# dblanm/gnn-manip

Hardware: AMD Instinct MI355X
Metric: rollout steps/sec (N particles, 10 MP steps, hidden=128) (higher is better)
Workload: dtype f32; 1 GPU; north_star target: N=100k dense synthetic scene, conn_r=0.015, max_neighbours=20, hidden=128, 10 MP steps; n_particles=100000, hidden=128, edges_last_step=1966056, k_steps=6, candidates_per_gpu=1, parallelism=candidate-parallel x1

## Files before the change

### gnn_manip_amd/csrc/hedge.hip

```cpp
#include <type_traits>
#include "common.h"
#include "mlp.h"
#include "hedge.h"
#include "hmlp.h"
#include "hmma_dev.h"
#include "blocks_dev.h"

namespace gm {

namespace {

constexpr int H = 128;
constexpr int BE = 32;
constexpr int SYS_THREADS = 768;
static_assert(BE == kBlockEdges, "block tables and the systolic kernels agree on the block size");
#ifdef HEDGE_STAMPS
__device__ unsigned long long g_sys_stamps[3 * 32 * 8 + 32];
#define SYS_STAMP(tick, slot)                                                                                         \
    do {                                                                                                              \
        if (blockIdx.x == 0 && jb == 0 && lane0 == 0 && (tick) >= 16 && (tick) < 48) {                                \
            g_sys_stamps[(role * 32 + (tick) - 16) * 8 + (slot)] = __builtin_readcyclecounter();                     \
            if (role == 0 && (slot) == 0) g_sys_stamps[3 * 32 * 8 + (tick) - 16] = __builtin_amdgcn_s_memrealtime(); \
        }                                                                                                             \
    } while (0)
#else
#define SYS_STAMP(tick, slot) do { } while (0)
#endif
constexpr int ST_STREAM_E = 2 | 16, ST_STREAM_AGG = 16;
constexpr int ST_ENC_E = 0;
constexpr int ST_PROJ_Q = 16;
constexpr int LD_SC1 = 16;
constexpr int HW_HEADER_FLOATS = 4;
constexpr int HW_VEC_FLOATS = 5 * H;
constexpr int HW_IMAGE_HALF8 = 3 * 4 * 8 * 2 * 64;


constexpr int TILE_ROW_B = 144;
constexpr int TILE_B = 32 * TILE_ROW_B;
constexpr int IMG_B = 16384;
constexpr int L_E = 0;
constexpr int L_X1 = L_E + 2 * IMG_B;
constexpr int L_X2 = L_X1 + 2 * IMG_B;
constexpr int L_Z = L_X2 + 2 * IMG_B;
constexpr int L_PS = L_Z + 8 * TILE_B;
constexpr int L_ST = L_PS + 4 * TILE_B;
constexpr int L_KM = L_ST + 2 * 32 * 4 * 4;
constexpr int L_KM2 = L_KM + 4 * 32 * 4;
constexpr int L_ZERO_END = L_KM2 + 4 * 32 * 4;
constexpr int L_VEC = L_ZERO_END;
constexpr int DR_SLOTS = 8;
constexpr int L_DR = L_VEC + 4 * H * 4;
constexpr size_t SYS_LDS_BYTES = L_DR + DR_SLOTS * BE * 4;
static_assert(SYS_LDS_BYTES <= 160 * 1024, "LDS budget");

__device__ __forceinline__ int eslot(int n, int kg, int ksbit) { return (n ^ (2 * (ksbit + 2 * kg))) + 32 * kg; }

typedef __amdgpu_buffer_rsrc_t srd_t;
__device__ __forceinline__ srd_t make_srd(const void* base, unsigned bytes) { return __builtin_amdgcn_make_buffer_rsrc(const_cast<void*>(base), 0, bytes, 0x00020000); }
__device__ __forceinline__ floatx4 bld4(srd_t r, unsigned voff, unsigned soff) { return __builtin_bit_cast(floatx4, __builtin_amdgcn_raw_buffer_load_b128(r, voff, soff, 0)); }
template <int NT>
__device__ __forceinline__ floatx4 bld4s(srd_t r, unsigned voff, unsigned soff) { return __builtin_bit_cast(floatx4, __builtin_amdgcn_raw_buffer_load_b128(r, voff, soff, NT)); }
template <int NT>
__device__ __forceinline__ void bst4s(srd_t r, unsigned voff, unsigned soff, floatx4 v) { __builtin_amdgcn_raw_buffer_store_b128(__builtin_bit_cast(uintx4, v), r, voff, soff, NT); }
__device__ __forceinline__ intx4 bldi4(srd_t r, unsigned voff, unsigned soff) { return __builtin_bit_cast(intx4, __builtin_amdgcn_raw_buffer_load_b128(r, voff, soff, 0)); }
__device__ __forceinline__ void bst4(srd_t r, unsigned voff, unsigned soff, floatx4 v) { __builtin_amdgcn_raw_buffer_store_b128(__builtin_bit_cast(uintx4, v), r, voff, soff, 0); }
template <int AUX>
__device__ __forceinline__ void bst1s(srd_t r, unsigned voff, unsigned soff, float v) { __builtin_amdgcn_raw_buffer_store_b32(__float_as_uint(v), r, voff, soff, AUX); }
__device__ __forceinline__ int xcd_major_wg() {
    const int g = (int)gridDim.x, i = (int)blockIdx.x;
    return (g & 7) == 0 ? (i & 7) * (g >> 3) + (i >> 3) : i;
}

__device__ __forceinline__ int s_clamp0(int v, int hi) {
    int r;
    asm("s_max_i32 %0, %1, 0\n\ts_min_i32 %0, %0, %2" : "=s"(r) : "s"(v), "s"(hi) : "scc");
    return r;
}

extern __shared__ __attribute__((aligned(16))) char smem[];
#define LDS(T, off) (*reinterpret_cast<T*>(smem + (off)))
__device__ __forceinline__ unsigned opaque(unsigned v) { asm volatile("" : "+v"(v)); return v; }
__device__ __forceinline__ int tick_no(int t) { asm volatile("" : "+s"(t)); return t; }
#define GM_SB __builtin_amdgcn_sched_barrier(0)

template <int NP>
__device__ __forceinline__ void acc_to_image(const floatx16& a, char* smem, unsigned addr) {
#pragma unroll
    for (int q = 0; q < 2; ++q) {
        float v[8];
#pragma unroll
        for (int j = 0; j < 8; ++j) v[j] = relu(a[8 * q + j]);
        uintx2 h0, l0, h1, l1;
        if constexpr (NP == 3) {
            split4(v[0], v[1], v[2], v[3], h0, l0);
            split4(v[4], v[5], v[6], v[7], h1, l1);
        } else {
            hi4(v[0], v[1], v[2], v[3], h0);
            hi4(v[4], v[5], v[6], v[7], h1);
        }
        LDS(uintx4, addr + (q * 2 + 0) * 1024) = uintx4{h0[0], h0[1], h1[0], h1[1]};
        if constexpr (NP == 3) LDS(uintx4, addr + (q * 2 + 1) * 1024) = uintx4{l0[0], l0[1], l1[0], l1[1]};
    }
}

template <int NP, class F>
__device__ __forceinline__ void mlp_layer(floatx16& acc, const floatx16& c0, const half8 (&wh)[8], const half8 (&wl)[8], char* smem, unsigned a0, unsigned a1, F&& side) {
    if constexpr (NP == 1) {
        half8 bh = LDS(half8, a0);
#pragma unroll
        for (int ks = 0; ks < 8; ++ks) {
            half8 nh = bh;
            const unsigned an = (((ks + 1) & 1) ? a1 : a0) + (ks + 1) * 2048;
            GM_SB;
            acc = __builtin_amdgcn_mfma_f32_32x32x16_f16(wh[ks], bh, ks == 0 ? c0 : acc, 0, 0, 0);
            GM_SB;
            if (ks + 1 < 8) nh = LDS(half8, an);
            side(3 * ks);
            GM_SB;
            side(3 * ks + 1);
            GM_SB;
            side(3 * ks + 2);
            bh = nh;
        }
        GM_SB;
        return;
    }
    half8 bh = LDS(half8, a0), bl = LDS(half8, a0 + 1024);
#pragma unroll
    for (int ks = 0; ks < 8; ++ks) {
        half8 nh = bh;
        const unsigned an = (((ks + 1) & 1) ? a1 : a0) + (ks + 1) * 2048;
        GM_SB;
        acc = __builtin_amdgcn_mfma_f32_32x32x16_f16(wl[ks], bh, ks == 0 ? c0 : acc, 0, 0, 0);
        GM_SB;
        if (ks + 1 < 8) nh = LDS(half8, an);
        side(3 * ks);
        GM_SB;
        acc = __builtin_amdgcn_mfma_f32_32x32x16_f16(wh[ks], bl, acc, 0, 0, 0);
        GM_SB;
        if (ks + 1 < 8) bl = LDS(half8, an + 1024);
        side(3 * ks + 1);
        GM_SB;
        acc = __builtin_amdgcn_mfma_f32_32x32x16_f16(wh[ks], bh, acc, 0, 0, 0);
        GM_SB;
        side(3 * ks + 2);
        bh = nh;
    }
    GM_SB;
}

__device__ __forceinline__ float ln_k(char* smem, unsigned st, float inv_T, float eps) {
    const float q = (LDS(float, st) + LDS(float, st + 128)) + (LDS(float, st + 256) + LDS(float, st + 384));
    const float v = fmaf(q * (1.0f / 128.0f) * inv_T, inv_T, eps);
    float r = __builtin_amdgcn_rsqf(v);
    r = r * fmaf(-0.5f * v * r, r, 1.5f);
    return inv_T * r;
}

__device__ __forceinline__ float lower_half_to_both(float v) {
    const auto r = __builtin_amdgcn_permlane32_swap(__float_as_uint(v), __float_as_uint(v), false, false);
    return __uint_as_float(r[0]);
}
__device__ __forceinline__ float upper_half_to_both(float v) {
    const auto r = __builtin_amdgcn_permlane32_swap(__float_as_uint(v), __float_as_uint(v), false, false);
    return __uint_as_float(r[1]);
}
__device__ __forceinline__ float sum_of_halves(float v) {
    const auto r = __builtin_amdgcn_permlane32_swap(__float_as_uint(v), __float_as_uint(v), false, false);
    return __uint_as_float(r[0]) + __uint_as_float(r[1]);
}

template <int R>
__device__ __forceinline__ void scan3_t(float& ya, float& yb, float& yc, float yprev, unsigned cont) {
    asm volatile("s_bfe_i32 exec_lo, %4, %5\n\ts_bfe_i32 exec_hi, %4, %6\n\tv_add_f32 %0, %0, %3\n\t"
                 "s_bfe_i32 exec_lo, %4, %7\n\ts_bfe_i32 exec_hi, %4, %8\n\tv_add_f32 %1, %1, %0\n\t"
                 "s_bfe_i32 exec_lo, %4, %9\n\ts_bfe_i32 exec_hi, %4, %10\n\tv_add_f32 %2, %2, %1\n\t"
                 "s_mov_b64 exec, -1"
                 : "+v"(ya), "+v"(yb), "+v"(yc)
                 : "v"(yprev), "s"(cont), "n"(0x10000 | R), "n"(0x10000 | (16 + R)), "n"(0x10000 | (R + 1)), "n"(0x10000 | (17 + R)),
// ... 335 lines not shown
        const unsigned km_rq = opaque(L_KM2 + jb * 128 + 64 * hi);
        const unsigned z_w = opaque(L_Z + jb * TILE_B + n * TILE_ROW_B + hi * 16);
        const unsigned z_t = opaque(L_Z + jb * TILE_B + 16 * hi * TILE_ROW_B + n * 4);
        const unsigned x_in = opaque(L_X2 + lane0 * 16);
        const unsigned dr_r = opaque(L_DR + 64 * hi);
        const srd_t srd_agg = make_srd(reinterpret_cast<const char*>(a_agg) - L_ST, a_agg_bytes + L_ST);
        floatx16 b3v = vec_to_acc(smem, L_VEC, H, jb, hi);
        auto fetch = [&](int x, int2 bi, int2 si, int hd, int& st, int& cnt, int& fl, unsigned& cont, unsigned& last, int& head) {
            st = bi.x;
            if (!ok(x)) { cnt = 0; fl = 0; cont = 0; last = 0; return; }
            cnt = bi.y & 0xff;
            fl = bi.y >> 8;
            cont = (unsigned)si.x;
            last = (unsigned)si.y;
            if (fl & 1) head = hd;
        };
        auto tick_as = [&](auto par_c, auto kind_c, int t) __attribute__((always_inline)) {
            constexpr int PAR = decltype(par_c)::value, P2 = PAR, P3 = 1 - PAR;
            constexpr int KIND = decltype(kind_c)::value;
            const int x = b0 + t;
            const int2 bn_n = a_blk[clampb(x)], sn_n = a_seg[clampb(x)];
            const int hd_n = a_head[clampb(x - 1) >> 2];
            if constexpr (KIND == TICK_IDLE) {
                cnt_a = cnt_b; fl_a = fl_b; cont_a = cont_b; last_a = last_b;
                if (fl_b & 1) head_a = head_b;
                st_a = st_b;
                fetch(x - 1, bn, sn, hd_n, st_b, cnt_b, fl_b, cont_b, last_b, head_b);
                bn = bn_n;
                sn = sn_n;
                lds_barrier();
                return;
            }
            b3v = vec_to_acc(smem, L_VEC, H, jb, hi);
            const bool agg_on = ok(x - 3);
            SYS_STAMP(t, 0);
            LDS(float, v_aoff + (L_KM2 - L_ST)) = ln_k(smem, st_r + P3 * 512, inv_T, a_eps);
            SYS_STAMP(t, 1);
            const unsigned cont = agg_on ? cont_a : 0u, last = agg_on ? last_a : 0u;
            const int cnt_st = agg_on ? cnt_a : 0;
            const unsigned rel_a = (unsigned)(st_a - e0), rel_b = (unsigned)(st_b - e0);
            floatx16 y;
            floatx4 kq;
            float zz[4];
            LnGroup lg;
            float cpend = 0.f;
            auto side = [&](int slot) {
                if (slot < 8) {
                    const int c = slot >> 1;
                    if (!(slot & 1)) {
                        kq = LDS(floatx4, km_rq + 16 * c);
#pragma unroll
                        for (int i = 0; i < 4; ++i) zz[i] = LDS(float, z_t + P3 * 4 * TILE_B + (4 * c + i) * TILE_ROW_B);
                    } else {
#pragma unroll
                        for (int i = 0; i < 4; ++i) y[4 * c + i] = fmaf(zz[i] * kq[i], gam, bet);
                    }
                } else if (slot < 13) {
                    const int r = 3 * (slot - 8) + 1;
                    float ya = y[r], yb = y[r + 1], yc = y[r + 2];
                    const float yp = y[r - 1];
                    scan3(ya, yb, yc, yp, cont, r);
                    y[r] = ya; y[r + 1] = yb; y[r + 2] = yc;
                } else if (slot == 13) {
                    const float c0v = (cont & 1u) ? carry : 0.f;
                    const float open0 = y[15] + ((last & 0xffffu) ? 0.f : c0v);
                    const float from0 = lower_half_to_both(open0);
                    const float c1v = (cont & 0x10000u) ? from0 : 0.f;
                    cpend = hi ? c1v : c0v;
                } else if (WRITE_E && slot >= 14 && slot < 20) {
                    const int j = 1 + ((slot - 14) >> 1);
                    if (!((slot - 14) & 1)) {
                        lg.load(km_re + j * 32, z_e + P3 * 4 * TILE_B + j * 8 * TILE_ROW_B);
                    } else {
                        const floatx4 gmq = LDS(floatx4, L_VEC + (2 * H + 32 * jb + 4 * cq) * 4);
                        const floatx4 btq = LDS(floatx4, L_VEC + (3 * H + 32 * jb + 4 * cq) * 4);
                        lg.store<STREAM ? ST_STREAM_E : 0>(e_out_wg, rel_a, j, cnt_st, v_eoff, gmq, btq, er[j - 1], res_w, srd_ein, rel_b);
                    }
                }
            };
            SYS_STAMP(t, 2);
            auto stores = [&]() {
                unsigned pend = (last | (last >> 16)) & 0xffffu;
                const unsigned side_row = (a_side_off + (unsigned)(((x - 3) >> 2) * H)) * 4u;
                const unsigned drp = dr_r + ((x - 3) & (DR_SLOTS - 1)) * (BE * 4);
                while (pend) {
                    const int r = __builtin_ctz(pend);
                    pend &= pend - 1;
                    const unsigned long long mk = (unsigned long long)(0u - ((last >> r) & 1u)) | ((unsigned long long)(0u - ((last >> (16 + r)) & 1u)) << 32);
                    if (__builtin_amdgcn_inverse_ballot_w64(mk)) {
                        const int d = LDS(int, drp + 4 * r);
                        const unsigned off = (d == head_a ? side_row : (unsigned)d * (H * 4u)) + v_aoff;
                        bst1s<STREAM ? ST_STREAM_AGG : 0>(srd_agg, off, 0, y[r] + cpend);
                        cpend = 0.f;
                    }
                }
                const float nc = upper_half_to_both(y[15] + cpend);
                carry = (((last >> 31) & 1u) || !agg_on || cnt_a < BE) ? 0.f : nc;
            };
            if constexpr (KIND == TICK_DRAIN) {
#pragma unroll
                for (int slot = 0; slot < 20; ++slot) side(slot);
            } else {
            mlp_layer<NP>(acc, b3v, wh, wl, smem, x_in + P2 * IMG_B, x_in + P2 * IMG_B, side);
            SYS_STAMP(t, 3);
            rng |= __any(row_bad<NP>(acc[0])) ? 1 : 0;
            {
                float q = 0.f;
#pragma unroll
                for (int r = 0; r < 16; ++r) q = fmaf(acc[r], acc[r], q);
                LDS(float, v_aoff + P2 * 512) = sum_of_halves(q);
#pragma unroll
                for (int g = 0; g < 4; ++g) {
                    floatx4 z;
#pragma unroll
                    for (int tt = 0; tt < 4; ++tt) z[tt] = acc[4 * g + tt];
                    LDS(floatx4, z_w + P2 * 4 * TILE_B + 32 * g) = z;
                }
            }
            }
            SYS_STAMP(t, 4);
            stores();
            cnt_a = cnt_b; fl_a = fl_b; cont_a = cont_b; last_a = last_b;
            if (fl_b & 1) head_a = head_b;
            st_a = st_b;
            fetch(x - 1, bn, sn, hd_n, st_b, cnt_b, fl_b, cont_b, last_b, head_b);
            bn = bn_n;
            sn = sn_n;
            SYS_STAMP(t, 5);
            lds_barrier();
            SYS_STAMP(t, 6);
        };
        auto tick = [&](auto par_c, int t) __attribute__((always_inline)) { tick_as(par_c, int_c<TICK_FULL>{}, t); };
        tick_as(int_c<1>{}, int_c<TICK_IDLE>{}, -1);
        tick_as(int_c<0>{}, int_c<TICK_IDLE>{}, 0);
        tick_as(int_c<1>{}, int_c<TICK_IDLE>{}, 1);
        tick(int_c<0>{}, tick_no(2));
        RUN_TICKS(3, nb - 1, tick);
        tick(int_c<1>{}, nb + 1);
        tick_as(int_c<0>{}, int_c<TICK_DRAIN>{}, nb + 2);
        report_split_range<false>(rng, lane0, a_flags);
    }
}

constexpr int LE_X1 = 0;
constexpr int LE_X2 = LE_X1 + 2 * IMG_B;
constexpr int LE_Z = LE_X2 + 2 * IMG_B;
constexpr int LE_ST = LE_Z + 8 * TILE_B;
constexpr int LE_KM = LE_ST + 2 * 4 * 32 * 4;
constexpr int RS_SLOTS = 8;
constexpr int LE_RS = LE_KM + 4 * 32 * 4;
constexpr int LE_ZERO_END = LE_RS + RS_SLOTS * 32 * 4;
constexpr int LE_VEC = LE_ZERO_END;
constexpr size_t ENC_LDS_BYTES = LE_VEC + 5 * H * 4;

template <int NP>
__global__ void __launch_bounds__(SYS_THREADS, 1) sys_enc_kernel(const CsrHeader* a_hdr, const float* __restrict__ a_x, float* __restrict__ a_e_out,
                                                                      const float* __restrict__ a_hw, int* a_flags, float a_eps, int a_pad_rows) {
    const int tid = threadIdx.x, lane0 = tid & 63;
    const int wave = __builtin_amdgcn_readfirstlane(tid >> 6);
    const int role = wave >> 2, jb = wave & 3;
    const int E = a_hdr->n_edges;
    const int nblk = (E + BE - 1) / BE;
    const int2 br = wg_range(nblk, true);
    const int b0 = br.x, b1 = br.y;
    const int nb = b1 - b0;
    if (a_pad_rows && blockIdx.x == 0)
        for (int i = tid; i < kEdgePadRows * H / 4; i += SYS_THREADS) reinterpret_cast<floatx4*>(a_e_out + (size_t)E * H)[i] = floatx4{0.f, 0.f, 0.f, 0.f};
    if (nb <= 0) return;
    const float inv_T = a_hw[1], cap = a_hw[2];
    half8 wh[8], wl[8];
    sys_prologue<NP>(wh, wl, reinterpret_cast<const half8*>(a_hw + HW_HEADER_FLOATS + HW_VEC_FLOATS), role * 4 + jb, role == 0, LE_ZERO_END, LE_VEC,
                      a_hw + HW_HEADER_FLOATS, 5 * H);
    const int n = lane0 & 31, hi = lane0 >> 5, rr = lane0 >> 3, cq = lane0 & 7;
    const int e0 = b0 * BE;
    const int rows_wg = (b1 * BE < E ? b1 * BE : E) - e0;
    floatx16 bv;
    {
        const int slot = role == 0 ? 4 : role - 1;
#pragma unroll
        for (int g = 0; g < 4; ++g) {
            const floatx4 v = LDS(floatx4, LE_VEC + (slot * H + 32 * jb + 4 * hi + 8 * g) * 4);
#pragma unroll
            for (int tt = 0; tt < 4; ++tt) bv[4 * g + tt] = v[tt];
        }
    }
    const unsigned rs_l = opaque(LE_RS + n * 4);
    int rng = 0;
    floatx16 acc;
    auto scaled_bias = [&](float sc) {
        floatx16 c;
#pragma unroll
        for (int r = 0; r < 16; ++r) c[r] = bv[r] * sc;
        return c;
    };
    if (role == 0) {
        const srd_t srd_x = make_srd(a_x + (size_t)e0 * 4, (unsigned)(rows_wg > 0 ? rows_wg : 0) * 16u);
        float* const e_out_wg = a_e_out + (size_t)e0 * H;
        const unsigned v_xoff = opaque(n * 16 + (hi ? 0x40000000u : 0u));
        const unsigned v_eoff = opaque(rr * 512 + jb * 128 + cq * 16);
        const unsigned x1_w = opaque(LE_X1 + 4 * jb * 1024 + lane0 * 16);
        const unsigned st_r = opaque(LE_ST + n * 4);
        const unsigned km_w = opaque(LE_KM + jb * 128 + n * 4), km_r = opaque(LE_KM + jb * 128 + rr * 4);
        const unsigned z_r = opaque(LE_Z + jb * TILE_B + rr * TILE_ROW_B + cq * 16);
        const floatx4 gm = LDS(floatx4, LE_VEC + (2 * H + 32 * jb + 4 * cq) * 4);
        const floatx4 bt = LDS(floatx4, LE_VEC + (3 * H + 32 * jb + 4 * cq) * 4);
        const float T3 = 1.0f / inv_T;
        floatx4 xq = bld4(srd_x, v_xoff, 0);
        auto tick = [&](auto par_c, int t) {
            constexpr int PAR = decltype(par_c)::value, P3 = 1 - PAR;
            const int x = b0 + t;
            float mx = fmaxf(fmaxf(fabsf(xq[0]), fabsf(xq[1])), fmaxf(fabsf(xq[2]), fabsf(xq[3])));
            float sc = cap;
            if (mx > 0.f && mx < 3.0e38f) {
                int ex;
                (void)frexpf(mx, &ex);
                sc = fminf(ldexpf(1.f, min(7 - ex, 100)), cap);
            }
            sc = lower_half_to_both(sc);
            if (jb == 0 && hi == 0) LDS(float, rs_l + (x & (RS_SLOTS - 1)) * 128) = sc;
            uintx2 h, l;
            if constexpr (NP == 3) split4(xq[0] * sc, xq[1] * sc, xq[2] * sc, xq[3] * sc, h, l);
            else hi4(xq[0] * sc, xq[1] * sc, xq[2] * sc, xq[3] * sc, h);
            const half8 bh = __builtin_bit_cast(half8, uintx4{h[0], h[1], 0u, 0u});
            const floatx16 c0v = scaled_bias(sc);
            {
                const int xn = x + 1 < b0 ? b0 : (x + 1 < b1 ? x + 1 : b1 - 1);
                xq = bld4(srd_x, v_xoff, (unsigned)(xn - b0) * 512u);
            }
            if constexpr (NP == 3) {
            const half8 bl = __builtin_bit_cast(half8, uintx4{l[0], l[1], 0u, 0u});
            acc = __builtin_amdgcn_mfma_f32_32x32x16_f16(wl[0], bh, c0v, 0, 0, 0);
            acc = __builtin_amdgcn_mfma_f32_32x32x16_f16(wh[0], bl, acc, 0, 0, 0);
            acc = __builtin_amdgcn_mfma_f32_32x32x16_f16(wh[0], bh, acc, 0, 0, 0);
            } else {
                acc = __builtin_amdgcn_mfma_f32_32x32x16_f16(wh[0], bh, c0v, 0, 0, 0);
            }
            {
                const float rs3 = LDS(float, rs_l + ((x - 3) & (RS_SLOTS - 1)) * 128);
                const float q = (LDS(float, st_r + P3 * 512) + LDS(float, st_r + P3 * 512 + 128)) + (LDS(float, st_r + P3 * 512 + 256) + LDS(float, st_r + P3 * 512 + 384));
                const float tt3 = T3 * rs3;
                const float v = fmaf(a_eps * tt3, tt3, q * (1.0f / 128.0f));
                float r = __builtin_amdgcn_rsqf(v);
                r = r * fmaf(-0.5f * v * r, r, 1.5f);
                LDS(float, km_w) = r;
                const int xb = x - 3;
                const int cnt = (xb >= b0 && xb < b1) ? min(BE, E - xb * BE) : 0;
#pragma unroll
                for (int j = 0; j < 4; ++j) {
                    const float kr = LDS(float, km_r + j * 32);
                    const floatx4 zq = LDS(floatx4, z_r + P3 * 4 * TILE_B + j * 8 * TILE_ROW_B);
                    floatx4 o;
#pragma unroll
                    for (int tt = 0; tt < 4; ++tt) o[tt] = fmaf(zq[tt] * kr, gm[tt], bt[tt]);
                    bst4s<ST_ENC_E>(make_srd(e_out_wg + (size_t)((xb - b0) * BE + 8 * j) * H, (unsigned)s_clamp0(cnt - 8 * j, 8) * 512u), v_eoff, 0, o);
                }
            }
            rng |= __any(row_bad<NP>(acc[0])) ? 1 : 0;
            GM_SB;
            acc_to_image<NP>(acc, smem, x1_w + PAR * IMG_B);
            lds_barrier();
        };
        RUN_TICKS(0, nb + 2, tick);
    } else if (role == 1) {
        const unsigned x_in = opaque(LE_X1 + lane0 * 16), x_out = opaque(LE_X2 + 4 * jb * 1024 + lane0 * 16);
        auto nothing = [](int) {};
        auto tick = [&](auto par_c, int t) {
            constexpr int PAR = decltype(par_c)::value, P1 = 1 - PAR;
            const int x = b0 + t;
            const floatx16 c0v = scaled_bias(LDS(float, rs_l + ((x - 1) & (RS_SLOTS - 1)) * 128));
            mlp_layer<NP>(acc, c0v, wh, wl, smem, x_in + P1 * IMG_B, x_in + P1 * IMG_B, nothing);
            rng |= __any(row_bad<NP>(acc[0])) ? 1 : 0;
            GM_SB;
            acc_to_image<NP>(acc, smem, x_out + P1 * IMG_B);
            lds_barrier();
        };
        RUN_TICKS(0, nb + 2, tick);
    } else {
        const unsigned x_in = opaque(LE_X2 + lane0 * 16);
        const unsigned st_w = opaque(LE_ST + jb * 128 + n * 4);
        const unsigned z_w = opaque(LE_Z + jb * TILE_B + n * TILE_ROW_B + hi * 16);
        auto nothing = [](int) {};
        auto tick = [&](auto par_c, int t) {
            constexpr int PAR = decltype(par_c)::value, P2 = PAR;
            const int x = b0 + t;
            const floatx16 c0v = scaled_bias(LDS(float, rs_l + ((x - 2) & (RS_SLOTS - 1)) * 128));
            mlp_layer<NP>(acc, c0v, wh, wl, smem, x_in + P2 * IMG_B, x_in + P2 * IMG_B, nothing);
            rng |= __any(row_bad<NP>(acc[0])) ? 1 : 0;
            publish_ln_stats(acc, st_w + P2 * 512, z_w + P2 * 4 * TILE_B);
            lds_barrier();
        };
        RUN_TICKS(0, nb + 2, tick);
    }
    report_split_range(rng, lane0, a_flags);
}

constexpr int LN_E = 0;
constexpr int LN_X1 = LN_E + 2 * IMG_B;
constexpr int LN_X2 = LN_X1 + 2 * IMG_B;
constexpr int LN_Z = LN_X2 + 2 * IMG_B;
constexpr int LN_PS = LN_Z + 8 * TILE_B;
constexpr int LN_ST = LN_PS + 4 * TILE_B;
constexpr int LN_KM = LN_ST + 2 * 4 * 32 * 4;
constexpr int LN_ZERO_END = LN_KM + 2 * 4 * 32 * 4;
constexpr int LN_VEC = LN_ZERO_END;
constexpr size_t NODE_LDS_BYTES = LN_VEC + 4 * H * 4;
static_assert(NODE_LDS_BYTES <= 160 * 1024, "LDS budget");

template <int NP>
__device__ __forceinline__ void sys_node_body(const float* a_h, const float* __restrict__ a_agg, const float* __restrict__ a_Q,
                                              float* a_h_out, const float* __restrict__ a_hw, int a_n, int* a_flags, float a_eps) {
    const int tid = threadIdx.x, lane0 = tid & 63;
    const int wave = __builtin_amdgcn_readfirstlane(tid >> 6);
    const int role = wave >> 2, jb = wave & 3;
    const int N = a_n;
    const int nblk = (N + BE - 1) / BE;
    const int wg = (int)blockIdx.x;
    const int b0 = (int)((long long)wg * nblk / gridDim.x), b1 = (int)((long long)(wg + 1) * nblk / gridDim.x);
    const int nb = b1 - b0;
    if (nb <= 0) return;
    const float inv_T = a_hw[1];
    half8 wh[8], wl[8];
    sys_prologue<NP>(wh, wl, reinterpret_cast<const half8*>(a_hw + HW_HEADER_FLOATS + HW_VEC_FLOATS), role * 4 + jb, false, LN_ZERO_END, LN_VEC,
                 a_hw + HW_HEADER_FLOATS, 4 * H);
    const int n = lane0 & 31, hi = lane0 >> 5, rr = lane0 >> 3, cq = lane0 & 7;
    const int r0 = b0 * BE;
    const int rows_wg = (b1 * BE < N ? b1 * BE : N) - r0;
    const unsigned wg_bytes = (unsigned)(rows_wg > 0 ? rows_wg : 0) * 512u;
    const unsigned v_eoff = opaque(rr * 512 + jb * 128 + cq * 16);
    int rng = 0;
    set_role_prio(role);
    if (role == 0) {
        const srd_t srd_q = make_srd(a_Q + (size_t)r0 * H, wg_bytes), srd_a = make_srd(a_agg + (size_t)r0 * H, wg_bytes);
        const unsigned v_qoff = opaque(rr * 2048 + jb * 128 + cq * 16);
        const unsigned ps_w = opaque(LN_PS + jb * TILE_B + 4 * rr * TILE_ROW_B + cq * 16);
        const unsigned ps_r = opaque(LN_PS + jb * TILE_B + n * TILE_ROW_B + hi * 16);
        const int kg = cq & 1, ksb = cq >> 2, half = (cq >> 1) & 1;
        const unsigned e_w = opaque(LN_E + ((2 * jb + ksb) * 2 * 64 + ((rr ^ (2 * (ksb + 2 * kg))) + 32 * kg)) * 16 + half * 8);
        const unsigned e_r0 = opaque(LN_E + eslot(n, hi, 0) * 16), e_r1 = opaque(LN_E + eslot(n, hi, 1) * 16);
        const unsigned x1_w = opaque(LN_X1 + 4 * jb * 1024 + lane0 * 16);
        floatx4 qv[4], eq[4];
#pragma unroll
        for (int j = 0; j < 4; ++j) { qv[j] = floatx4{0.f, 0.f, 0.f, 0.f}; eq[j] = bld4(srd_a, v_eoff, j * 4096); }
        floatx16 acc, c0v;
#pragma unroll
        for (int r = 0; r < 16; ++r) c0v[r] = 0.f;
        auto clampb = [&](int x) { return x < b0 ? b0 : (x < b1 ? x : b1 - 1); };
        auto tick_as = [&](auto par_c, auto kind_c, int t) {
            constexpr int PAR = decltype(par_c)::value, KIND = decltype(kind_c)::value;
            if constexpr (KIND == TICK_DRAIN) {
                lds_barrier();
                return;
            }
            const int x = b0 + t;
            const unsigned rel1 = (unsigned)(clampb(x + 1) - b0) * (BE * 512u), rel2 = (unsigned)(clampb(x + 2) - b0) * (BE * 512u);
#pragma unroll
            for (int j = 0; j < 4; ++j) qv[j] = bld4(srd_q, v_qoff, rel1 + j * 512);
            auto side = [&](int slot) {
                if (slot < 8 && !(slot & 1)) {
                    const int j = slot >> 1;
                    uintx2 h, l;
                    if constexpr (NP == 3) split4(eq[j][0], eq[j][1], eq[j][2], eq[j][3], h, l);
                    else hi4(eq[j][0], eq[j][1], eq[j][2], eq[j][3], h);
                    LDS(uintx2, e_w + (1 - PAR) * IMG_B + j * 128) = h;
                    if constexpr (NP == 3) LDS(uintx2, e_w + (1 - PAR) * IMG_B + j * 128 + 1024) = l;
                } else if (slot == 8) {
#pragma unroll
                    for (int j = 0; j < 4; ++j) eq[j] = bld4(srd_a, v_eoff, rel2 + j * 4096);
                }
            };
            if constexpr (KIND == TICK_FULL) {
                mlp_layer<NP>(acc, c0v, wh, wl, smem, e_r0 + PAR * IMG_B, e_r1 + PAR * IMG_B, side);
                rng |= __any(row_bad<NP>(acc[0])) ? 1 : 0;
                GM_SB;
                acc_to_image<NP>(acc, smem, x1_w + PAR * IMG_B);
            } else {
#pragma unroll
                for (int slot = 0; slot <= 8; ++slot) side(slot);
            }
#pragma unroll
            for (int j = 0; j < 4; ++j) LDS(floatx4, ps_w + j * TILE_ROW_B) = qv[j];
#pragma unroll
            for (int g = 0; g < 4; ++g) {
                const floatx4 v = LDS(floatx4, ps_r + 32 * g);
#pragma unroll
                for (int tt = 0; tt < 4; ++tt) c0v[4 * g + tt] = v[tt];
            }
            lds_barrier();
        };
        NODE_TICKS(tick_as);
    } else {
        const bool r2 = role == 2;
        const int eg0 = r2 ? 2 : 0;
        const srd_t srd_h = make_srd(a_h + (size_t)r0 * H, wg_bytes);
        float* const h_out_wg = a_h_out + (size_t)r0 * H;
        const floatx4 gm = LDS(floatx4, LN_VEC + (2 * H + 32 * jb + 4 * cq) * 4);
        const floatx4 bt = LDS(floatx4, LN_VEC + (3 * H + 32 * jb + 4 * cq) * 4);
        const floatx16 bv = vec_to_acc(smem, LN_VEC, r2 ? H : 0, jb, hi);
        const unsigned st_r = opaque(LN_ST + n * 4);
        const unsigned km_w = opaque(LN_KM + (r2 ? 512 : 0) + jb * 128 + n * 4), km_r = opaque(LN_KM + (r2 ? 512 : 0) + jb * 128 + rr * 4);
        const unsigned z_r = opaque(LN_Z + jb * TILE_B + rr * TILE_ROW_B + cq * 16);
        const unsigned x_in = opaque((r2 ? LN_X2 : LN_X1) + lane0 * 16), x_out = opaque(LN_X2 + 4 * jb * 1024 + lane0 * 16);
        const unsigned st_w = opaque(LN_ST + jb * 128 + n * 4);
        const unsigned z_w = opaque(LN_Z + jb * TILE_B + n * TILE_ROW_B + hi * 16);
        floatx4 er[2];
        er[0] = er[1] = floatx4{0.f, 0.f, 0.f, 0.f};
        floatx16 acc;
        auto tick_as = [&](auto par_c, auto kind_c, int t) {
            constexpr int PAR = decltype(par_c)::value, PIN = 1 - PAR, P3 = 1 - PAR;
            constexpr int KIND = decltype(kind_c)::value;
            if constexpr (KIND == TICK_FILL) {
                lds_barrier();
                return;
            }
            const int x = b0 + t;
            LDS(float, km_w) = ln_k(smem, st_r + P3 * 512, inv_T, a_eps);
            const int xb = x - 3;
            const int cnt = (xb >= b0 && xb < b1) ? min(BE, N - xb * BE) : 0;
            const unsigned rel_a = (unsigned)((xb < b0 ? b0 : xb) - b0) * BE;
            const int xr = x - 2 < b0 ? b0 : (x - 2 < b1 ? x - 2 : b1 - 1);
            const unsigned rel_b = (unsigned)(xr - b0) * (BE * 512u);
            float kr;
            floatx4 zq;
            auto side = [&](int slot) {
                if (slot != 0 && slot != 2 && slot != 6 && slot != 8) return;
                const int jj = slot >= 6, j = eg0 + jj;
                if (slot == 0 || slot == 6) {
                    kr = LDS(float, km_r + j * 32);
                    zq = LDS(floatx4, z_r + P3 * 4 * TILE_B + j * 8 * TILE_ROW_B);
                } else {
                    floatx4 o;
#pragma unroll
                    for (int tt = 0; tt < 4; ++tt) o[tt] = er[jj][tt] + fmaf(zq[tt] * kr, gm[tt], bt[tt]);
                    bst4(make_srd(h_out_wg + (size_t)(rel_a + 8 * j) * H, (unsigned)s_clamp0(cnt - 8 * j, 8) * 512u), v_eoff, 0, o);
                    er[jj] = bld4(srd_h, v_eoff, rel_b + j * 4096);
                }
            };
            if constexpr (KIND == TICK_DRAIN) {
#pragma unroll
                for (int slot = 0; slot <= 8; ++slot) side(slot);
            } else if (!r2) {
                mlp_layer<NP>(acc, bv, wh, wl, smem, x_in + PIN * IMG_B, x_in + PIN * IMG_B, side);
                rng |= __any(row_bad<NP>(acc[0])) ? 1 : 0;
                GM_SB;
                acc_to_image<NP>(acc, smem, x_out + PIN * IMG_B);
// ... 322 lines not shown
        }
        hipLaunchKernelGGL(pack_h3_kernel, dim3(J.n), dim3(H3_PACK_THREADS), 0, s, J);
        GM_LAUNCH_CHECK();
    }
    return GM_OK;
}

static size_t max_blocks_of(int64_t n_nodes, int64_t edge_capacity) {
    return (size_t)cdiv(edge_capacity, BE) + 4 * (size_t)n_nodes + 4;
}
size_t edge_groups_max(int64_t n_nodes, int64_t edge_capacity) { return max_blocks_of(n_nodes, edge_capacity) / 4 + 1 + kSinkRows; }

size_t edge_blocks_ints(int64_t n_nodes, int64_t edge_capacity) {
    const size_t nblk = max_blocks_of(n_nodes, edge_capacity);
    return 8 + ((size_t)n_nodes + 2) + 1 + 4 * nblk + (nblk / 4 + 2) + 2 * (size_t)n_nodes;
}

EdgeBlocks carve_edge_blocks(int* base, int64_t n_nodes, int64_t edge_capacity) {
    EdgeBlocks t;
    const size_t nblk = max_blocks_of(n_nodes, edge_capacity);
    t.hdr = reinterpret_cast<EdgeBlockHeader*>(base);
    t.gblk = base + 8;
    int* p = t.gblk + n_nodes + 2;
    p += (reinterpret_cast<uintptr_t>(p) & 4) ? 1 : 0;
    t.blk = reinterpret_cast<int2*>(p);
    t.seg = reinterpret_cast<int2*>(p + 2 * nblk);
    t.head = p + 4 * nblk;
    t.stitch = t.head + nblk / 4 + 2;
    t.stitch_list = t.stitch + n_nodes;
    t.max_blocks = (int64_t)nblk;
    return t;
}

int build_edge_blocks(const int* in_ptr, const int* dst, int64_t n_nodes, const int* n_per_graph_dev, int n_per_graph_host, const EdgeBlocks& t, hipStream_t s) {
    hipLaunchKernelGGL(edge_blocks_plan_kernel, dim3(1), dim3(64), 0, s, in_ptr, (int)n_nodes, n_per_graph_dev, n_per_graph_host,
                       t.hdr, t.gblk, (int)n_nodes + 1);
    int gb = (int)cdiv(t.max_blocks, 256);
    gb = gb < 1 ? 1 : (gb > 1024 ? 1024 : gb);
    hipLaunchKernelGGL(edge_blocks_fill_kernel, dim3(gb), dim3(256), 0, s, in_ptr, dst, (int)n_nodes, t.hdr, t.gblk, t.blk, t.seg, t.head, t.stitch,
                       t.stitch_list);
    GM_LAUNCH_CHECK();
    return GM_OK;
}

bool edge_sys_fits(int64_t n_nodes, int64_t edge_capacity) {
    const uint64_t agg_rows = (uint64_t)n_nodes + edge_groups_max(n_nodes, edge_capacity);
    return (uint64_t)n_nodes * 2 * H * 4 < (1ull << 32) && agg_rows * H * 4 < (1ull << 32);
}

constexpr uint64_t kStreamStoreBytes = 128ull << 20;

template <auto KERNEL, class... Args>
static int launch_sys(size_t lds, ProfState* prof_state, int kind, hipStream_t s, Args... args) {
    static PerDeviceOnce attr_done;
    const int rc_attr = attr_done.run([lds]() -> int {
        GM_HIP_CHECK(hipFuncSetAttribute(reinterpret_cast<const void*>(KERNEL), hipFuncAttributeMaxDynamicSharedMemorySize, (int)lds));
        return GM_OK;
    });
    if (rc_attr != GM_OK) return rc_attr;
    {
        ProfScope prof(prof_state, kind, s);
        hipLaunchKernelGGL(KERNEL, dim3(device_cus()), dim3(SYS_THREADS), lds, s, args...);
    }
    GM_LAUNCH_CHECK();
    return GM_OK;
}
template <auto KERNEL>
using kernel_c = std::integral_constant<decltype(KERNEL), KERNEL>;
int launch_edge_sys(const EdgeArgs& a, const EdgeBlocks& t, int64_t edge_capacity, hipStream_t s) {
    GM_REQUIRE(a.hdr && a.wstream_h3 && a.agg && a.side && !a.eid && !a.eid_out, GM_ERR_INVALID_ARGUMENT, "launch_edge_sys: unsupported argument combination");
    GM_REQUIRE(a.P_prescaled, GM_ERR_INVALID_ARGUMENT, "launch_edge_sys: P must carry the weight scale of this step (HmNodeArgs::p_scale = edge_sys_p_scale(image))");
    const uint64_t agg_bytes = ((uint64_t)(a.side - a.agg) + (uint64_t)(t.max_blocks / 4 + 1) * H) * 4;
    GM_REQUIRE(a.side >= a.agg && agg_bytes < (1ull << 32) && (uint64_t)a.n_nodes_tab * 2 * H * 4 < (1ull << 32), GM_ERR_INVALID_ARGUMENT,
               "launch_edge_sys: P and agg + side buffer must each stay below 4 GiB (edge_sys_fits)");
    const bool stream = (uint64_t)edge_capacity * H * 4 > kStreamStoreBytes;
    auto go = [&](auto kern) {
        return launch_sys<decltype(kern)::value>(SYS_LDS_BYTES, a.prof, PROF_EDGE, s, a.hdr, a.dst, a.src, a.P, a.e_in, a.e_out, a.agg, a.wstream_h3,
                                                 t.blk, t.seg, t.head, t.hdr, (unsigned)(a.side - a.agg), (unsigned)agg_bytes,
                                                 (unsigned)((uint64_t)a.n_nodes_tab * 2 * H * 4), const_cast<int*>(&a.hdr->error_flags), a.eps, a.residual);
    };
    auto pick = [&](auto np_c) {
        constexpr int NP = decltype(np_c)::value;
        if (a.discard_e_out) return stream ? go(kernel_c<sys_edge_kernel<false, true, NP>>{}) : go(kernel_c<sys_edge_kernel<false, false, NP>>{});
        return stream ? go(kernel_c<sys_edge_kernel<true, true, NP>>{}) : go(kernel_c<sys_edge_kernel<true, false, NP>>{});
    };
    return a.precision == kPrecisionF16 ? pick(int_c<NP_F16>{}) : pick(int_c<NP_F32>{});
}

int launch_edge_sys_enc(const EdgeArgs& a, hipStream_t s) {
    GM_REQUIRE(a.hdr && a.wstream_h3 && a.e_in && a.e_out && !a.eid && !a.eid_out && a.k1 == 4, GM_ERR_INVALID_ARGUMENT,
               "launch_edge_sys_enc: unsupported argument combination");
    auto go = [&](auto kern) {
        return launch_sys<decltype(kern)::value>(ENC_LDS_BYTES, a.prof, PROF_ENC, s, a.hdr, a.e_in, a.e_out, a.wstream_h3, const_cast<int*>(&a.hdr->error_flags),
                                                 a.eps, a.zero_pad_rows ? 1 : 0);
    };
    return a.precision == kPrecisionF16 ? go(kernel_c<sys_enc_kernel<NP_F16>>{}) : go(kernel_c<sys_enc_kernel<NP_F32>>{});
}

int launch_node_sys(const NodeSysArgs& a, hipStream_t s) {
    GM_REQUIRE(a.h && a.agg && a.Q && a.h_out && a.image && a.n > 0, GM_ERR_INVALID_ARGUMENT, "launch_node_sys: bad argument");
    auto go = [&](auto kern) {
        return launch_sys<decltype(kern)::value>(NODE_LDS_BYTES, a.prof, PROF_NODE, s, a.h, a.agg, a.Q, a.h_out, a.image, a.n, a.flags, a.eps);
    };
    return a.precision == kPrecisionF16 ? go(kernel_c<sys_node_kernel<NP_F16>>{}) : go(kernel_c<sys_node_kernel<NP_F32>>{});
}

int launch_proj_sys(const ProjSysArgs& a, hipStream_t s) {
    GM_REQUIRE(a.h && a.P && a.Q && a.img_p && a.img_q && a.n > 0, GM_ERR_INVALID_ARGUMENT, "launch_proj_sys: bad argument");
    auto go = [&](auto kern) {
        return launch_sys<decltype(kern)::value>(PROJ_LDS_BYTES, a.prof, PROF_NODE, s, a.h, a.P, a.Q, a.img_p, a.img_q, a.scale_p, a.scale_q, a.n, a.flags);
    };
    return a.precision == kPrecisionF16 ? go(kernel_c<sys_proj_kernel<NP_F16>>{}) : go(kernel_c<sys_proj_kernel<NP_F32>>{});
}

int launch_node_proj_sys(const NodeSysArgs& a, const ProjSysArgs& p, hipStream_t s) {
    GM_REQUIRE(a.h && a.agg && a.Q && a.h_out && a.image && a.n > 0, GM_ERR_INVALID_ARGUMENT, "launch_node_proj_sys: bad argument");
    GM_REQUIRE(p.P && p.img_p && p.img_q, GM_ERR_INVALID_ARGUMENT, "launch_node_proj_sys: bad argument");
    GM_REQUIRE(p.h == a.h_out && p.Q == a.Q && p.n == a.n && p.flags == a.flags, GM_ERR_INVALID_ARGUMENT,
               "launch_node_proj_sys: the projection must read the node MLP's h_out and write its Q, over the same rows");
    GM_REQUIRE(p.precision == a.precision, GM_ERR_INVALID_ARGUMENT, "launch_node_proj_sys: the two halves disagree on the precision");
    auto go = [&](auto kern) {
        return launch_sys<decltype(kern)::value>(NODE_PROJ_LDS_BYTES, a.prof, PROF_NODE, s, a.h, a.h_out, a.agg, p.Q, a.image, p.P, p.img_p, p.img_q,
                                                 p.scale_p, p.scale_q, a.n, a.flags, a.eps);
    };
    return a.precision == kPrecisionF16 ? go(kernel_c<sys_node_proj_kernel<NP_F16>>{}) : go(kernel_c<sys_node_proj_kernel<NP_F32>>{});
}

int launch_agg_stitch(float* agg, const float* side, const EdgeBlocks& t, int64_t n, ProfState* prof_state, hipStream_t s) {
    if (n <= 0) return GM_OK;
    {
        ProfScope prof(prof_state, PROF_NODE, s);
        int64_t gb = cdiv(n * 8, 256 * 4);
        gb = gb < 1 ? 1 : (gb > 2048 ? 2048 : gb);
        hipLaunchKernelGGL(agg_stitch_kernel, dim3((unsigned)gb), dim3(256), 0, s, agg, side, t.stitch, t.stitch_list, t.head, t.hdr, (int)n);
    }
    GM_LAUNCH_CHECK();
    return GM_OK;
}

__global__ void __launch_bounds__(256) edge_pad_rows_kernel(const CsrHeader* hdr, float* e, int row_floats) {
    const size_t base = (size_t)hdr->n_edges * row_floats;
    for (int i = blockIdx.x * blockDim.x + threadIdx.x; i < kEdgePadRows * row_floats; i += gridDim.x * blockDim.x) e[base + i] = 0.f;
}
int zero_edge_pad_rows(const CsrHeader* hdr, float* e, int row_floats, hipStream_t s) {
    hipLaunchKernelGGL(edge_pad_rows_kernel, dim3(4), dim3(256), 0, s, hdr, e, row_floats);
    GM_LAUNCH_CHECK();
    return GM_OK;
}

#ifdef HEDGE_STAMPS
extern "C" int gm_debug_sys_stamps(unsigned long long* out) {
    return hipMemcpyFromSymbol(out, HIP_SYMBOL(g_sys_stamps), sizeof(unsigned long long) * (3 * 32 * 8 + 32)) == hipSuccess ? 0 : -1;
}
#endif

}
```

Measured before the change: 128.5 rollout steps/s.

## Deepen edge-encoder systolic pipeline to overlap MLP epilogues with next block's MFMA chain

The three-role edge-encoder kernel moves from a 3-stage to a 5-stage software pipeline. Roles 1 and 2 keep double-buffered accumulators, so the relu/convert/LDS-store epilogue (or the LayerNorm statistics) of the previous block is interleaved as side work inside the next block's MFMA chain. This hides epilogue latency behind matrix ops. In exchange it adds register pressure from two floatx16 accumulators, deeper fill and drain ticks, more complex tick scheduling macros, and debug stamps that are compiled out by default.

```diff
diff --git a/gnn_manip_amd/csrc/hedge.hip b/gnn_manip_amd/csrc/hedge.hip
--- a/gnn_manip_amd/csrc/hedge.hip
+++ b/gnn_manip_amd/csrc/hedge.hip
@@ -23,8 +23,15 @@
             if (role == 0 && (slot) == 0) g_sys_stamps[3 * 32 * 8 + (tick) - 16] = __builtin_amdgcn_s_memrealtime(); \
         }                                                                                                             \
     } while (0)
+__device__ unsigned long long g_enc_stamps[3 * 32 * 8];
+#define ENC_STAMP(tick, slot)                                                                                         \
+    do {                                                                                                              \
+        if (blockIdx.x == 0 && jb == 0 && lane0 == 0 && (tick) >= 16 && (tick) < 48)                                  \
+            g_enc_stamps[(role * 32 + (tick) - 16) * 8 + (slot)] = __builtin_readcyclecounter();                     \
+    } while (0)
 #else
 #define SYS_STAMP(tick, slot) do { } while (0)
+#define ENC_STAMP(tick, slot) do { } while (0)
 #endif
 constexpr int ST_STREAM_E = 2 | 16, ST_STREAM_AGG = 16;
 constexpr int ST_ENC_E = 0;
@@ -666,6 +673,43 @@
 constexpr int LE_ZERO_END = LE_RS + RS_SLOTS * 32 * 4;
 constexpr int LE_VEC = LE_ZERO_END;
 constexpr size_t ENC_LDS_BYTES = LE_VEC + 5 * H * 4;
+static_assert(ENC_LDS_BYTES <= 160 * 1024, "LDS budget");
+constexpr int ENC_DEPTH = 5;
+static_assert(ENC_DEPTH + 1 <= RS_SLOTS, "the scale ring holds every block in flight");
+
+#define ENC_T(tick_as, par, ch, tl, t) tick_as(int_c<(par)>{}, std::bool_constant<(ch)>{}, std::bool_constant<(tl)>{}, t)
+#define ENC_DRAIN(tick_as, C, D, p0)                                \
+    ENC_T(tick_as, (p0), 0 < (C), 0 < (D), nb);                     \
+    ENC_T(tick_as, 1 - (p0), 1 < (C), 1 < (D), nb + 1);             \
+    ENC_T(tick_as, (p0), 2 < (C), 2 < (D), nb + 2);                 \
+    ENC_T(tick_as, 1 - (p0), 3 < (C), 3 < (D), nb + 3);             \
+    ENC_T(tick_as, (p0), 4 < (C), 4 < (D), nb + 4);
+#define ENC_TICKS(tick_as, C, D)                                                                        \
+    if (nb >= ENC_DEPTH) {                                                                              \
+        ENC_T(tick_as, 0, 0 >= (C), 0 >= (D), 0);                                                       \
+        ENC_T(tick_as, 1, 1 >= (C), 1 >= (D), 1);                                                       \
+        ENC_T(tick_as, 0, 2 >= (C), 2 >= (D), 2);                                                       \
+        ENC_T(tick_as, 1, 3 >= (C), 3 >= (D), 3);                                                       \
+        ENC_T(tick_as, 0, 4 >= (C), 4 >= (D), 4);                                                       \
+        int t_ = ENC_DEPTH;                                                                             \
+        _Pragma("unroll 1") for (; t_ + 1 < nb; t_ += 2) {                                              \
+            ENC_T(tick_as, 1, true, true, t_);                                                          \
+            ENC_T(tick_as, 0, true, true, t_ + 1);                                                      \
+        }                                                                                               \
+        if (t_ < nb) {              \
+            ENC_T(tick_as, 1, true, true, t_);                                                          \
+            ENC_DRAIN(tick_as, C, D, 0)                                                                 \
+        } else {                                                                                        \
+            ENC_DRAIN(tick_as, C, D, 1)                                                                 \
+        }                                                                                               \
+    } else {                                                                                            \
+        _Pragma("unroll 1") for (int t_ = 0; t_ < nb + ENC_DEPTH; t_ += 2) {                            \
+            tick_as(int_c<0>{}, t_ >= (C) && t_ < (C) + nb, t_ >= (D) && t_ < (D) + nb, t_);            \
+            if (t_ + 1 < nb + ENC_DEPTH)                                                                \
+                tick_as(int_c<1>{}, t_ + 1 >= (C) && t_ + 1 < (C) + nb, t_ + 1 >= (D) && t_ + 1 < (D) + nb, t_ + 1); \
+        }                                                                                               \
+    }
+static_assert(ENC_DEPTH == 5, "ENC_TICKS and ENC_DRAIN spell out five fill and five drain ticks");
 
 template <int NP>
 __global__ void __launch_bounds__(SYS_THREADS, 1) sys_enc_kernel(const CsrHeader* a_hdr, const float* __restrict__ a_x, float* __restrict__ a_e_out,
@@ -700,14 +744,16 @@
     }
     const unsigned rs_l = opaque(LE_RS + n * 4);
     int rng = 0;
-    floatx16 acc;
+    floatx16 acc2[2];
     auto scaled_bias = [&](float sc) {
         floatx16 c;
 #pragma unroll
         for (int r = 0; r < 16; ++r) c[r] = bv[r] * sc;
         return c;
     };
+    auto nothing = [](int) {};
     if (role == 0) {
+        floatx16& acc = acc2[0];
         const srd_t srd_x = make_srd(a_x + (size_t)e0 * 4, (unsigned)(rows_wg > 0 ? rows_wg : 0) * 16u);
         float* const e_out_wg = a_e_out + (size_t)e0 * H;
         const unsigned v_xoff = opaque(n * 16 + (hi ? 0x40000000u : 0u));
@@ -720,9 +766,12 @@
         const floatx4 bt = LDS(floatx4, LE_VEC + (3 * H + 32 * jb + 4 * cq) * 4);
         const float T3 = 1.0f / inv_T;
         floatx4 xq = bld4(srd_x, v_xoff, 0);
-        auto tick = [&](auto par_c, int t) {
+        auto tick_as = [&](auto par_c, auto ch, auto ep, int t) __attribute__((always_inline)) {
             constexpr int PAR = decltype(par_c)::value, P3 = 1 - PAR;
+            constexpr bool FULL = std::is_same_v<decltype(ch), bool>;
             const int x = b0 + t;
+            ENC_STAMP(t, 0);
+            if (FULL || ch) {
             float mx = fmaxf(fmaxf(fabsf(xq[0]), fabsf(xq[1])), fmaxf(fabsf(xq[2]), fabsf(xq[3])));
             float sc = cap;
             if (mx > 0.f && mx < 3.0e38f) {
@@ -749,15 +798,17 @@
             } else {
                 acc = __builtin_amdgcn_mfma_f32_32x32x16_f16(wh[0], bh, c0v, 0, 0, 0);
             }
-            {
-                const float rs3 = LDS(float, rs_l + ((x - 3) & (RS_SLOTS - 1)) * 128);
+            }
+            ENC_STAMP(t, 1);
+            if (FULL || ep) {
+                const float rs3 = LDS(float, rs_l + ((x - ENC_DEPTH) & (RS_SLOTS - 1)) * 128);
                 const float q = (LDS(float, st_r + P3 * 512) + LDS(float, st_r + P3 * 512 + 128)) + (LDS(float, st_r + P3 * 512 + 256) + LDS(float, st_r + P3 * 512 + 384));
                 const float tt3 = T3 * rs3;
                 const float v = fmaf(a_eps * tt3, tt3, q * (1.0f / 128.0f));
                 float r = __builtin_amdgcn_rsqf(v);
                 r = r * fmaf(-0.5f * v * r, r, 1.5f);
                 LDS(float, km_w) = r;
-                const int xb = x - 3;
+                const int xb = x - ENC_DEPTH;
                 const int cnt = (xb >= b0 && xb < b1) ? min(BE, E - xb * BE) : 0;
 #pragma unroll
                 for (int j = 0; j < 4; ++j) {
@@ -769,41 +820,102 @@
                     bst4s<ST_ENC_E>(make_srd(e_out_wg + (size_t)((xb - b0) * BE + 8 * j) * H, (unsigned)s_clamp0(cnt - 8 * j, 8) * 512u), v_eoff, 0, o);
                 }
             }
-            rng |= __any(row_bad<NP>(acc[0])) ? 1 : 0;
-            GM_SB;
-            acc_to_image<NP>(acc, smem, x1_w + PAR * IMG_B);
+            if (FULL || ch) {
+                rng |= __any(row_bad<NP>(acc[0])) ? 1 : 0;
+                GM_SB;
+                acc_to_image<NP>(acc, smem, x1_w + PAR * IMG_B);
+            }
+            ENC_STAMP(t, 2);
             lds_barrier();
+            ENC_STAMP(t, 3);
         };
-        RUN_TICKS(0, nb + 2, tick);
+        ENC_TICKS(tick_as, 0, ENC_DEPTH)
     } else if (role == 1) {
         const unsigned x_in = opaque(LE_X1 + lane0 * 16), x_out = opaque(LE_X2 + 4 * jb * 1024 + lane0 * 16);
-        auto nothing = [](int) {};
-        auto tick = [&](auto par_c, int t) {
+        auto tick_as = [&](auto par_c, auto ch, auto tl, int t) __attribute__((always_inline)) {
             constexpr int PAR = decltype(par_c)::value, P1 = 1 - PAR;
+            constexpr bool BOTH = std::is_same_v<decltype(ch), std::true_type> && std::is_same_v<decltype(tl), std::true_type>;
             const int x = b0 + t;
-            const floatx16 c0v = scaled_bias(LDS(float, rs_l + ((x - 1) & (RS_SLOTS - 1)) * 128));
-            mlp_layer<NP>(acc, c0v, wh, wl, smem, x_in + P1 * IMG_B, x_in + P1 * IMG_B, nothing);
-            rng |= __any(row_bad<NP>(acc[0])) ? 1 : 0;
-            GM_SB;
-            acc_to_image<NP>(acc, smem, x_out + P1 * IMG_B);
+            ENC_STAMP(t, 0);
+            const floatx16& ta = acc2[P1];
+            float ra = 0.f, rb = 0.f;
+            unsigned hh[4] = {0u, 0u, 0u, 0u}, ll[4] = {0u, 0u, 0u, 0u};
+            auto tail = [&](int s) __attribute__((always_inline)) {
+                const int p = s / 3, k = p & 3, q = p >> 2;
+                if (s % 3 == 0) {
+                    ra = relu(ta[2 * p]);
+                    rb = relu(ta[2 * p + 1]);
+                    hh[k] = cvt_pk(ra, rb);
+                } else if (s % 3 == 1) {
+                    if constexpr (NP == 3) ll[k] = lo_pair(hh[k], ra, rb);
+                } else if (k == 3) {
+                    LDS(uintx4, x_out + PAR * IMG_B + (q * 2 + 0) * 1024) = uintx4{hh[0], hh[1], hh[2], hh[3]};
+                    if constexpr (NP == 3) LDS(uintx4, x_out + PAR * IMG_B + (q * 2 + 1) * 1024) = uintx4{ll[0], ll[1], ll[2], ll[3]};
+                }
+            };
+            auto chain = [&](auto&& side) __attribute__((always_inline)) {
+                const floatx16 c0v = scaled_bias(LDS(float, rs_l + ((x - 1) & (RS_SLOTS - 1)) * 128));
+                mlp_layer<NP>(acc2[PAR], c0v, wh, wl, smem, x_in + P1 * IMG_B, x_in + P1 * IMG_B, side);
+                rng |= __any(row_bad<NP>(acc2[PAR][0])) ? 1 : 0;
+            };
+            if constexpr (BOTH) {
+                chain(tail);
+                ENC_STAMP(t, 1);
+            } else {
+                if (ch) chain(nothing);
+                ENC_STAMP(t, 1);
+                if (tl) {
+                    GM_SB;
+#pragma unroll
+                    for (int s = 0; s < 24; ++s) tail(s);
+                }
+            }
+            ENC_STAMP(t, 2);
             lds_barrier();
+            ENC_STAMP(t, 3);
         };
-        RUN_TICKS(0, nb + 2, tick);
+        ENC_TICKS(tick_as, 1, 2)
     } else {
         const unsigned x_in = opaque(LE_X2 + lane0 * 16);
         const unsigned st_w = opaque(LE_ST + jb * 128 + n * 4);
         const unsigned z_w = opaque(LE_Z + jb * TILE_B + n * TILE_ROW_B + hi * 16);
-        auto nothing = [](int) {};
-        auto tick = [&](auto par_c, int t) {
-            constexpr int PAR = decltype(par_c)::value, P2 = PAR;
+        auto tick_as = [&](auto par_c, auto ch, auto tl, int t) __attribute__((always_inline)) {
+            constexpr int PAR = decltype(par_c)::value, P1 = 1 - PAR;
+            constexpr bool BOTH = std::is_same_v<decltype(ch), std::true_type> && std::is_same_v<decltype(tl), std::true_type>;
             const int x = b0 + t;
-            const floatx16 c0v = scaled_bias(LDS(float, rs_l + ((x - 2) & (RS_SLOTS - 1)) * 128));
-            mlp_layer<NP>(acc, c0v, wh, wl, smem, x_in + P2 * IMG_B, x_in + P2 * IMG_B, nothing);
-            rng |= __any(row_bad<NP>(acc[0])) ? 1 : 0;
-            publish_ln_stats(acc, st_w + P2 * 512, z_w + P2 * 4 * TILE_B);
+            ENC_STAMP(t, 0);
+            const floatx16& ta = acc2[P1];
+            float q = 0.f;
+            auto tail = [&](int s) __attribute__((always_inline)) {
+                if (s % 3 != 2) return;
+                const int k = s / 3, g = k >> 1;
+                q = fmaf(ta[2 * k], ta[2 * k], q);
+                q = fmaf(ta[2 * k + 1], ta[2 * k + 1], q);
+                if (k & 1) LDS(floatx4, z_w + PAR * 4 * TILE_B + 32 * g) = floatx4{ta[4 * g], ta[4 * g + 1], ta[4 * g + 2], ta[4 * g + 3]};
+                if (k == 7) LDS(float, st_w + PAR * 512) = sum_of_halves(q);
+            };
+            auto chain = [&](auto&& side) __attribute__((always_inline)) {
+                const floatx16 c0v = scaled_bias(LDS(float, rs_l + ((x - 3) & (RS_SLOTS - 1)) * 128));
+                mlp_layer<NP>(acc2[PAR], c0v, wh, wl, smem, x_in + P1 * IMG_B, x_in + P1 * IMG_B, side);
+                rng |= __any(row_bad<NP>(acc2[PAR][0])) ? 1 : 0;
+            };
+            if constexpr (BOTH) {
+                chain(tail);
+                ENC_STAMP(t, 1);
+            } else {
+                if (ch) chain(nothing);
+                ENC_STAMP(t, 1);
+                if (tl) {
+                    GM_SB;
+#pragma unroll
+                    for (int s = 0; s < 24; ++s) tail(s);
+                }
+            }
+            ENC_STAMP(t, 2);
             lds_barrier();
+            ENC_STAMP(t, 3);
         };
-        RUN_TICKS(0, nb + 2, tick);
+        ENC_TICKS(tick_as, 3, 4)
     }
     report_split_range(rng, lane0, a_flags);
 }
@@ -1432,6 +1544,9 @@
 extern "C" int gm_debug_sys_stamps(unsigned long long* out) {
     return hipMemcpyFromSymbol(out, HIP_SYMBOL(g_sys_stamps), sizeof(unsigned long long) * (3 * 32 * 8 + 32)) == hipSuccess ? 0 : -1;
 }
+extern "C" int gm_debug_enc_stamps(unsigned long long* out) {
+    return hipMemcpyFromSymbol(out, HIP_SYMBOL(g_enc_stamps), sizeof(unsigned long long) * (3 * 32 * 8)) == hipSuccess ? 0 : -1;
+}
 #endif
 
 }
```

Result: no change. 129.0 rollout steps/s, median of 6 (+0.4%).
